# MDFahimAnjum/AliasFree-Diffusion-Models-PyTorch

Measured on AMD Instinct MI355X. Metric: train_step_images_per_sec, higher is better.
Workload: dtype f32; 1 GPU; CIFAR-10 32x32x3 synthetic, UNet variant=3 (Config D), batch 256/GPU, T=1000, AdamW lr 3e-4, random-init weights (seed 42); global_batch=256, parallelism=dp1, hip_graph=True, launch_mode=lanes

## Files before the change

aliasfree-diffusion-models-pytorch_amd/csrc/conv.hip:

```cpp
#include <cstdlib>
#include <algorithm>
#include "common.h"

namespace afd {

using f32x16 = __attribute__((ext_vector_type(16))) float;

static inline int gs_grid(long total, int block = 256) {
  long g = (total + block - 1) / block;
  return (int)(g < 1 ? 1 : (g > 65536 ? 65536 : g));
}

template <int KS>
__global__ void conv_direct_fwd(const float* __restrict__ x, const float* __restrict__ w, const float* __restrict__ bias,
                                const float* __restrict__ res, float* __restrict__ y,
                                int Cin, int Cout, int H, int W, int act, long total) {
  constexpr int T = KS * KS, R = KS / 2;
  for (long i = blockIdx.x * (long)blockDim.x + threadIdx.x; i < total; i += (long)gridDim.x * blockDim.x) {
    const int xx = i % W, yy = (i / W) % H;
    const long bc = i / ((long)W * H);
    const int co = bc % Cout; const long b = bc / Cout;
    float acc = bias ? bias[co] : 0.f;
    for (int ci = 0; ci < Cin; ++ci) {
      const float* xp = x + (b * Cin + ci) * (long)H * W;
// ... 564 lines not shown
    const int bn = threadIdx.x >> 2;
    if ((threadIdx.x & 3) == 0 && bn < BNo && n0 + bn < Cout) bias_part[(long)split * Cout + n0 + bn] = t;
  }
  float* out = part + (long)split * Cout * Cin * T;
  if (WK == 1) {
    if (!active) return;
    const int ci = c0 + cw + l31;
    if (ci < Cin) {
#pragma unroll
      for (int r = 0; r < 16; ++r) {
        const int n = n0 + nw + (r & 3) + 8 * (r >> 2) + 4 * half;
        if (n >= Cout) continue;
#pragma unroll
        for (int t = 0; t < T; ++t) out[((long)t * Cout + n) * Cin + ci] = acc[t][r];
      }
    }
  } else {
    float* red = smem;
    constexpr int NB = WNn * WCn;
#pragma unroll
    for (int t = 0; t < T; ++t) {
      __syncthreads();
#pragma unroll
      for (int r = 0; r < 16; ++r) red[(wv * 16 + r) * 64 + lane] = acc[t][r];
      __syncthreads();
      for (int idx = threadIdx.x; idx < NB * 1024; idx += NT_) {
        const int blk = idx / 1024, r = (idx / 64) % 16, ln = idx % 64;
        float v = 0.f;
#pragma unroll
        for (int k = 0; k < WK; ++k) v += red[((k * NB + blk) * 16 + r) * 64 + ln];
        const int bn = blk % WNn, bc = blk / WNn;
        const int n = n0 + bn * 32 + (r & 3) + 8 * (r >> 2) + 4 * (ln >> 5);
        const int ci = c0 + bc * 32 + (ln & 31);
        if (n < Cout && ci < Cin) out[((long)t * Cout + n) * Cin + ci] = v;
      }
    }
  }
}

__global__ __launch_bounds__(256) void wgrad_reduce(const float* __restrict__ part, float* __restrict__ dw, long n, int splits,
                                                    const float* __restrict__ bias_part, float* __restrict__ db, int nb,
                                                    int accumulate, int T) {
  __shared__ float red[8][33];
  const long i = (long)blockIdx.x * 32 + (threadIdx.x & 31);
  const int g = threadIdx.x >> 5;
  const bool isw = i < n;
  const long j = isw ? i : i - n;
  const long stride = isw ? n : nb;
  const float* __restrict__ src = isw ? part : bias_part;
  float s0 = 0.f, s1 = 0.f, s2 = 0.f, s3 = 0.f;
  if (i < n + nb) {
    int k = g;
    for (; k + 24 < splits; k += 32) {
      s0 += src[(long)k * stride + j]; s1 += src[(long)(k + 8) * stride + j];
      s2 += src[(long)(k + 16) * stride + j]; s3 += src[(long)(k + 24) * stride + j];
    }
    for (; k < splits; k += 8) s0 += src[(long)k * stride + j];
  }
  red[g][threadIdx.x & 31] = (s0 + s1) + (s2 + s3);
  __syncthreads();
  if (g == 0 && i < n + nb) {
    float t = 0.f;
#pragma unroll
    for (int k = 0; k < 8; ++k) t += red[k][threadIdx.x & 31];
    const long plane = n / T;
    float* o = isw ? dw + (j % plane) * T + j / plane : db + j;
    *o = accumulate ? *o + t : t;
  }
}

__global__ __launch_bounds__(256) void wgrad_reduce4(const float* __restrict__ part, float* __restrict__ dw, long n, int splits,
                                                     const float* __restrict__ bias_part, float* __restrict__ db, int nb,
                                                     int accumulate, int T) {
  __shared__ float4 red4[8][32];
  const int l = threadIdx.x & 31, g = threadIdx.x >> 5;
  const long wblocks = n >> 7;
  if (blockIdx.x < wblocks) {
    const long j = ((long)blockIdx.x << 7) + 4 * l;
    const float4* __restrict__ src = reinterpret_cast<const float4*>(part + j);
    const long stride = n >> 2;
    float4 s0 = {0.f, 0.f, 0.f, 0.f}, s1 = s0, s2 = s0, s3 = s0;
    int k = g;
    for (; k + 24 < splits; k += 32) {
      const float4 a = src[(long)k * stride], b = src[(long)(k + 8) * stride], c = src[(long)(k + 16) * stride],
                   d = src[(long)(k + 24) * stride];
      s0.x += a.x; s0.y += a.y; s0.z += a.z; s0.w += a.w;
      s1.x += b.x; s1.y += b.y; s1.z += b.z; s1.w += b.w;
      s2.x += c.x; s2.y += c.y; s2.z += c.z; s2.w += c.w;
      s3.x += d.x; s3.y += d.y; s3.z += d.z; s3.w += d.w;
    }
    for (; k < splits; k += 8) {
      const float4 a = src[(long)k * stride];
      s0.x += a.x; s0.y += a.y; s0.z += a.z; s0.w += a.w;
    }
    red4[g][l] = make_float4((s0.x + s1.x) + (s2.x + s3.x), (s0.y + s1.y) + (s2.y + s3.y), (s0.z + s1.z) + (s2.z + s3.z),
                             (s0.w + s1.w) + (s2.w + s3.w));
    __syncthreads();
    if (threadIdx.x < 128) {
      const int e = threadIdx.x;
      float t = 0.f;
#pragma unroll
      for (int q = 0; q < 8; ++q) t += reinterpret_cast<const float*>(&red4[q][e >> 2])[e & 3];
      const long je = ((long)blockIdx.x << 7) + e, plane = n / T;
      float* o = dw + (je % plane) * T + je / plane;
      *o = accumulate ? *o + t : t;
    }
  } else {
    __shared__ float red[8][33];
    const long j = (long)(blockIdx.x - wblocks) * 32 + l;
    float s0 = 0.f;
    if (j < nb)
      for (int k = g; k < splits; k += 8) s0 += bias_part[(long)k * nb + j];
    red[g][l] = s0;
    __syncthreads();
    if (g == 0 && j < nb) {
      float t = 0.f;
#pragma unroll
      for (int q = 0; q < 8; ++q) t += red[q][l];
      db[j] = accumulate ? db[j] + t : t;
    }
  }
}

int fold_launch(const afd_fold_desc* descs, int n, hipStream_t s);

struct FoldSink { afd_fold_desc* out; int n; };
static int launch_wgrad_reduce(const float* part, float* dw, long n, int slabs, const float* bp, float* db, int nb, int accumulate,
                               int T, hipStream_t s, FoldSink* sink) {
  afd_fold_desc d[2];
  int nd = 0;
  d[nd++] = afd_fold_desc{part, dw, n, n, n / T, (long)T, slabs, accumulate};
  if (nb > 0) d[nd++] = afd_fold_desc{bp, db, (long)nb, (long)nb, (long)nb, 1L, slabs, accumulate};
  if (sink) {
    for (int i = 0; i < nd; ++i) sink->out[sink->n++] = d[i];
    return AFD_OK;
  }
  return fold_launch(d, nd, s);
}

bool pw_launch(const float* in, const float* w, const float* bias, const float* res, float* out, int B, int K, int N, int P,
               int act, bool dgrad, hipStream_t s);
void pw_set_mode(int m);
int wino_plan(int B, int K, int N, int H, int W);
bool wino_conv(const float* x, const float* w, const float* bias, const float* res, float* y, float* U, int B, int K, int N, int H,
               int W, int act, bool dgrad, bool weights_ready, hipStream_t s);
void wino_set_mode(int m);
void wino_weights_launch(const float* w, float* Uf, float* Ud, int Cin, int Cout, int kinds, hipStream_t s);
bool bf3_ok(int B, int K, int N, int H, int W);
void bf3_set_mode(int m);
void direct_form_set(int m);
bool direct_form_is_bf3();
void h2_sk_set_mode(int m);
void h2_lds_set(int m);
void wino_weights_batched_launch(const afd_wino_desc* descs, const int* wg_desc, int n_wg, hipStream_t s);
void wino_set_grid(int g);
int wgrad_wino_plan(int B, int Cin, int Cout, int H, int W, int* bn, int* bk, int* cps, int* nchunks);
int wgrad_bf3_plan(int B, int Cin, int Cout, int H, int W, int* tps, int* ntiles);
int wgrad_bf3(const float* x, const float* dy, float* part, int B, int Cin, int Cout, int H, int W, hipStream_t s);
void wgrad_bf3_set_mode(int m);
void wgrad_arith_set(int m);
void wgrad_plan_target_set(long wgs);
bool wgrad_arith_is_bf3();
int wgrad_h2(const float* x, const float* dy, float* part, int B, int Cin, int Cout, int H, int W, hipStream_t s);
int pw_wgrad_h2(const float* x, const float* dy, float* part, float* bias_part, int B, int Cin, int Cout, int L, hipStream_t s);
bool ends_fwd(const float* x, const float* w, const float* bias, const float* res, float* y, int B, int Cin, int Cout, int H, int W,
              int ksize, int act, hipStream_t s);
bool ends_dgrad(const float* dy, const float* w, float* dx, int B, int Cin, int Cout, int H, int W, int ksize, hipStream_t s);
void ends_set_mode(int m);
int wgrad_cin3_plan(int B, int Cin, int Cout, int H, int W);
int wgrad_cin3(const float* x, const float* dy, float* part, int B, int Cin, int Cout, int H, int W, hipStream_t s);
void pw_wgrad_bf3_set_mode(int m);
int pw_wgrad_bf3_plan(int B, int Cin, int Cout, int L, int* sps, int* nsteps, int* nr, int* nt);
int pw_wgrad_bf3(const float* x, const float* dy, float* part, float* bias_part, int B, int Cin, int Cout, int L, hipStream_t s);
int wgrad_wino(const float* x, const float* dy, float* part, int B, int Cin, int Cout, int H, int W, hipStream_t s);
void wgrad_wino_set_mode(int m);

static inline bool use_mfma(int K, int N, int H, int W, int PT) { return N >= 8 && tile_ok(H, W, PT); }

static int g_conv_path = 0;

template <int T, bool DGRAD>
static int launch_mfma(const float* x, const float* w, const float* bias, const float* res, float* y,
                       int B, int K, int N, int H, int W, int act, hipStream_t s) {
  constexpr int KC = (T == 9) ? 8 : 32;
  const long P = (long)B * H * W;
  if (P * K >= (1L << 31) || (long)K * N * T >= (1L << 31)) return -1;
  const unsigned ptiles = (unsigned)((P + 127) / 128);
  const long wgs64 = (long)ptiles * ((N + 63) / 64), wgs32 = (long)ptiles * ((N + 31) / 32);
  bool use32 = N <= 32 || (wgs64 < 256 && wgs32 >= 256);
  const bool want_sk = g_conv_path == 2 || (g_conv_path == 0 && wgs64 < 256 && wgs32 < 256);
  if (g_conv_path == 1) use32 = N <= 32;
  if (want_sk && K >= 32 && tile_ok(H, W, 64)) {
    const TileGeom g = make_geom(H, W, 64, T == 9 ? 1 : 0);
    if (g.XS <= 256) {
      const size_t lds_main = sizeof(float) * (32 * (32 * T + 1) + (size_t)32 * g.XS);
      const size_t lds_red = sizeof(float) * 4 * 2 * 16 * 64;
      const size_t lds = lds_main > lds_red ? lds_main : lds_red;
      hipLaunchKernelGGL((conv_mfma_sk<T, DGRAD>), dim3((N + 31) / 32, (unsigned)((P + 63) / 64)), dim3(256), lds, s,
                         x, w, bias, res, y, B, K, N, H, W, act, g);
      return 0;
    }
  }
  const TileGeom g = make_geom(H, W, 128, T == 9 ? 1 : 0);
  if (g.XS > 512) return -1;
  int geo = 0;
  if (T == 1) geo = 5;
  else if (H == W && (W == 32 || W == 16 || W == 8 || W == 4)) geo = W == 32 ? 1 : (W == 16 ? 2 : (W == 8 ? 3 : 4));
  const size_t lds = 2 * sizeof(float) * ((use32 ? 32 : 64) * (KC * T + 1) + (size_t)KC * g.XS);
  const dim3 grid(use32 ? (N + 31) / 32 : (N + 63) / 64, ptiles);
#define AFD_CONV_LAUNCH(BN_, GEO_) hipLaunchKernelGGL((conv_mfma<T, DGRAD, BN_, KC, GEO_>), grid, dim3(256), lds, s, x, w, bias, res, y, B, K, N, H, W, act, g)
#define AFD_CONV_GEO(BN_)                                             \
  switch (geo) {                                                       \
    case 1: if constexpr (T == 9) { AFD_CONV_LAUNCH(BN_, 1); } break;  \
    case 2: if constexpr (T == 9) { AFD_CONV_LAUNCH(BN_, 2); } break;  \
    case 3: if constexpr (T == 9) { AFD_CONV_LAUNCH(BN_, 3); } break;  \
    case 4: if constexpr (T == 9) { AFD_CONV_LAUNCH(BN_, 4); } break;  \
    case 5: if constexpr (T == 1) { AFD_CONV_LAUNCH(BN_, 5); } break;  \
    default: AFD_CONV_LAUNCH(BN_, 0);                                  \
  }
  if (!use32) { AFD_CONV_GEO(64) } else { AFD_CONV_GEO(32) }
#undef AFD_CONV_GEO
#undef AFD_CONV_LAUNCH
  return 0;
}

static int g_wgrad_nw = 0;
struct WgradPlan { int wnn, wcn, wk, splits, slabs, nchunks, cps, npb; };
static inline WgradPlan wgrad_plan(int B, int Cin, int Cout, int H, int W, int ksize) {
  WgradPlan p;
  p.wnn = Cout > 32 ? 2 : 1;
  p.wcn = Cin > 32 ? 2 : 1;
  p.wk = 4 / (p.wnn * p.wcn);
  p.nchunks = (int)(((long)B * H * W + 63) / 64);
  const long tiles = (long)((Cout + 32 * p.wnn - 1) / (32 * p.wnn)) * ((Cin + 32 * p.wcn - 1) / (32 * p.wcn));
  static const long target = [] { const char* e = getenv("AFD_WG_TARGET"); return e ? atol(e) : 256L; }();
  long s = target / tiles;
  if (s < 1) s = 1;
  if (s > p.nchunks) s = p.nchunks;
  p.cps = (int)((p.nchunks + s - 1) / s);
  p.splits = (int)((p.nchunks + p.cps - 1) / p.cps);
  p.slabs = p.splits;
  const TileGeom g = make_geom(H, W, 64, ksize == 3 ? 1 : 0);
  const int need = (g.XS + 31) / 32;
  p.npb = ksize == 1 ? 2 : (need <= 4 ? 4 : (need <= 5 ? 5 : 8));
  return p;
}

template <int T, int WNn, int WCn, int NPB>
static void launch_wgrad(const float* x, const float* dy, float* part, float* bias_part, int B, int Cin, int Cout, int H, int W,
                         const WgradPlan& p, const TileGeom& g, hipStream_t s) {
  const int nw = g_wgrad_nw ? g_wgrad_nw : ((p.cps >= 8 || (p.cps >= 4 && H * W >= 256)) ? 8 : 4);
  size_t lds = sizeof(float) * ((size_t)32 * WNn * 65 + (size_t)32 * WCn * (g.XS | 1)) + sizeof(int) * 64;
  const size_t red = sizeof(float) * nw * 16 * 64;
  if (WNn * WCn < nw && lds < red) lds = red;
  const dim3 grid((Cout + 32 * WNn - 1) / (32 * WNn), (Cin + 32 * WCn - 1) / (32 * WCn), p.splits);
  if (nw == 8)
    hipLaunchKernelGGL((conv_wgrad_mfma<T, WNn, WCn, NPB, 8>), grid, dim3(512), lds, s, x, dy, part, bias_part, B, Cin, Cout, H, W, p.cps, p.nchunks, g);
  else
    hipLaunchKernelGGL((conv_wgrad_mfma<T, WNn, WCn, NPB, 4>), grid, dim3(256), lds, s, x, dy, part, bias_part, B, Cin, Cout, H, W, p.cps, p.nchunks, g);
}

template <int T, int NPB>
static void launch_wgrad_roles(const float* x, const float* dy, float* part, float* bp, int B, int Cin, int Cout, int H, int W,
                               const WgradPlan& p, const TileGeom& g, hipStream_t s) {
  if (p.wnn == 2 && p.wcn == 2) launch_wgrad<T, 2, 2, NPB>(x, dy, part, bp, B, Cin, Cout, H, W, p, g, s);
  else if (p.wnn == 2) launch_wgrad<T, 2, 1, NPB>(x, dy, part, bp, B, Cin, Cout, H, W, p, g, s);
  else if (p.wcn == 2) launch_wgrad<T, 1, 2, NPB>(x, dy, part, bp, B, Cin, Cout, H, W, p, g, s);
  else launch_wgrad<T, 1, 1, NPB>(x, dy, part, bp, B, Cin, Cout, H, W, p, g, s);
}

}
using namespace afd;

extern "C" {

int afd_debug_conv_path(int mode) {
  if (mode >= 92 && mode <= 93) { ends_set_mode(mode - 92); return AFD_OK; }
  if (mode >= 88 && mode <= 89) { pw_wgrad_bf3_set_mode(mode - 88); return AFD_OK; }
  if (mode >= 84 && mode <= 86) { wgrad_bf3_set_mode(mode - 84); return AFD_OK; }
  if (mode >= 48 && mode <= 49) { wgrad_plan_target_set(mode == 48 ? 256 : 160); return AFD_OK; }
  if (mode >= 59 && mode <= 63) { h2_lds_set(mode == 59 ? 4 : (mode == 60 ? 1 : (mode == 61 ? 0 : mode - 60))); return AFD_OK; }
  if (mode == 73) { h2_sk_set_mode(2); return AFD_OK; }
  if (mode >= 74 && mode <= 75) { h2_sk_set_mode(mode - 74); return AFD_OK; }
  if (mode >= 78 && mode <= 79) { wgrad_arith_set(mode - 78); return AFD_OK; }
  if (mode >= 76 && mode <= 77) { direct_form_set(mode - 76); return AFD_OK; }
  if (mode >= 80 && mode <= 82) { bf3_set_mode(mode - 80); return AFD_OK; }
  if (mode >= 8 && mode <= 10) { pw_set_mode(mode - 8); return AFD_OK; }
  if (mode >= 100000 && mode < 200000) { wino_set_grid(mode - 100000); return AFD_OK; }
  if (mode >= 96 && mode <= 98) { wgrad_wino_set_mode(mode - 96); return AFD_OK; }
  if (mode >= 64 && mode <= 70) { wino_set_mode(mode - 64); return AFD_OK; }
  if (mode >= 32 && mode <= 34) { g_wgrad_nw = mode == 32 ? 4 : (mode == 33 ? 8 : 0); return AFD_OK; }
  AFD_REQUIRE(mode >= 0 && mode <= 2, "afd_debug_conv_path: mode must be 0 (auto), 1 (big tile), 2 (split-K tile), 8..10 (1x1 streaming auto/off/forced), 32..34 (wgrad waves 4/8/auto), 64..69 (Winograd fwd/dgrad auto/off/forced shapes) or 96..98 (Winograd wgrad auto/off/forced)");
  g_conv_path = mode;
  return AFD_OK;
}

int afd_conv_fwd(const float* x, const float* w, const float* bias, const float* res, float* y,
                 int B, int Cin, int Cout, int H, int W, int ksize, int act, afd_stream_t st) {
  AFD_REQUIRE(x && w && y && B > 0 && Cin > 0 && Cout > 0 && H > 0 && W > 0, "afd_conv_fwd: bad argument");
  AFD_REQUIRE(ksize == 1 || ksize == 3, "afd_conv_fwd: ksize %d not in {1,3}", ksize);
  AFD_REQUIRE(act == 0 || act == 1, "afd_conv_fwd: act must be 0 or 1");
  hipStream_t s = as_stream(st);
  if (ends_fwd(x, w, bias, res, y, B, Cin, Cout, H, W, ksize, act, s)) return check_launch("afd_conv_fwd");
  if (ksize == 1 && pw_launch(x, w, bias, res, y, B, Cin, Cout, H * W, act, false, s)) return check_launch("afd_conv_fwd");
  int rc = -1;
  if (use_mfma(Cin, Cout, H, W, 128))
    rc = ksize == 3 ? launch_mfma<9, false>(x, w, bias, res, y, B, Cin, Cout, H, W, act, s)
                    : launch_mfma<1, false>(x, w, bias, res, y, B, Cin, Cout, H, W, act, s);
  if (rc != 0) {
    const long total = (long)B * Cout * H * W;
    if (ksize == 3) hipLaunchKernelGGL(conv_direct_fwd<3>, dim3(gs_grid(total)), dim3(256), 0, s, x, w, bias, res, y, Cin, Cout, H, W, act, total);
    else hipLaunchKernelGGL(conv_direct_fwd<1>, dim3(gs_grid(total)), dim3(256), 0, s, x, w, bias, res, y, Cin, Cout, H, W, act, total);
  }
  return check_launch("afd_conv_fwd");
}

int afd_conv_dgrad(const float* dy, const float* w, float* dx, int B, int Cin, int Cout, int H, int W, int ksize, afd_stream_t st) {
  AFD_REQUIRE(dy && w && dx && B > 0 && Cin > 0 && Cout > 0 && H > 0 && W > 0, "afd_conv_dgrad: bad argument");
  AFD_REQUIRE(ksize == 1 || ksize == 3, "afd_conv_dgrad: ksize %d not in {1,3}", ksize);
  hipStream_t s = as_stream(st);
  if (ends_dgrad(dy, w, dx, B, Cin, Cout, H, W, ksize, s)) return check_launch("afd_conv_dgrad");
  if (ksize == 1 && pw_launch(dy, w, nullptr, nullptr, dx, B, Cout, Cin, H * W, 0, true, s)) return check_launch("afd_conv_dgrad");
  int rc = -1;
  if (use_mfma(Cout, Cin, H, W, 128))
    rc = ksize == 3 ? launch_mfma<9, true>(dy, w, nullptr, nullptr, dx, B, Cout, Cin, H, W, 0, s)
                    : launch_mfma<1, true>(dy, w, nullptr, nullptr, dx, B, Cout, Cin, H, W, 0, s);
  if (rc != 0) {
    const long total = (long)B * Cin * H * W;
    if (ksize == 3) hipLaunchKernelGGL(conv_direct_dgrad<3>, dim3(gs_grid(total)), dim3(256), 0, s, dy, w, dx, Cin, Cout, H, W, total);
    else hipLaunchKernelGGL(conv_direct_dgrad<1>, dim3(gs_grid(total)), dim3(256), 0, s, dy, w, dx, Cin, Cout, H, W, total);
  }
  return check_launch("afd_conv_dgrad");
}

size_t afd_conv3x3_wino_workspace_bytes(int B, int Cin, int Cout, int H, int W, int dgrad) {
  if (B <= 0 || Cin <= 0 || Cout <= 0 || H <= 0 || W <= 0) return 0;
  const int K = dgrad ? Cout : Cin, N = dgrad ? Cin : Cout;
  return (bf3_ok(B, K, N, H, W) || wino_plan(B, K, N, H, W)) ? sizeof(float) * 16 * (size_t)Cin * Cout : 0;
}

int afd_conv3x3_weight_kinds(int B, int Cin, int Cout, int H, int W) {
  if (B <= 0 || Cin <= 0 || Cout <= 0 || H <= 0 || W <= 0) return 0;
  const int k = (bf3_ok(B, Cin, Cout, H, W) ? 1 : 0) | (bf3_ok(B, Cout, Cin, H, W) ? 2 : 0);
  return k && direct_form_is_bf3() ? k | 4 : k;
}

int afd_conv3x3_wino_weights(const float* w, float* u_fwd, float* u_dgrad, int Cin, int Cout, int kinds, afd_stream_t st) {
  AFD_REQUIRE(w && (u_fwd || u_dgrad) && Cin > 0 && Cout > 0 && Cin % 8 == 0 && Cout % 8 == 0, "afd_conv3x3_wino_weights: bad argument");
  AFD_REQUIRE(kinds >= 0 && kinds <= 7 && (!(kinds & 4) || (kinds & 3)) && (!(kinds & 3) || (Cin % 16 == 0 && Cout % 16 == 0)), "afd_conv3x3_wino_weights: bad kinds %d", kinds);
  wino_weights_launch(w, u_fwd, u_dgrad, Cin, Cout, kinds, as_stream(st));
  return check_launch("afd_conv3x3_wino_weights");
}

int afd_conv3x3_wino_weights_batched(const afd_wino_desc* descs, const int* wg_desc, int n_wg, afd_stream_t st) {
  AFD_REQUIRE(descs && wg_desc && n_wg > 0, "afd_conv3x3_wino_weights_batched: bad argument");
  wino_weights_batched_launch(descs, wg_desc, n_wg, as_stream(st));
  return check_launch("afd_conv3x3_wino_weights_batched");
}

static int check_kinds(const char* who, int kinds, int B, int Cin, int Cout, int H, int W, int dgrad) {
  const int now = afd_conv3x3_weight_kinds(B, Cin, Cout, H, W);
  const int bit = dgrad ? 2 : 1;
  AFD_REQUIRE(kinds >= 0 && (kinds & bit) == (now & bit) && (!(now & bit) || (kinds & 4) == (now & 4)),
              "%s: the weight image was built as kinds %d, but a call with (B %d, %d -> %d, %dx%d) under the current settings reads kinds %d "
              "(rebuild it: afd_conv3x3_weight_kinds depends on the batch size and on afd_debug_conv_path)", who, kinds, B, Cin, Cout, H, W, now);
  return AFD_OK;
}

int afd_conv3x3_wino_fwd(const float* x, const float* w, const float* bias, const float* res, float* y,
                         int B, int Cin, int Cout, int H, int W, int act, void* workspace, int weights_ready, int kinds, afd_stream_t st) {
  AFD_REQUIRE(x && w && y && workspace && B > 0 && Cin > 0 && Cout > 0 && H > 0 && W > 0, "afd_conv3x3_wino_fwd: bad argument");
  AFD_REQUIRE(act == 0 || act == 1, "afd_conv3x3_wino_fwd: act must be 0 or 1");
  if (weights_ready && check_kinds("afd_conv3x3_wino_fwd", kinds, B, Cin, Cout, H, W, 0) != AFD_OK) return AFD_EINVAL;
  AFD_REQUIRE(wino_conv(x, w, bias, res, y, static_cast<float*>(workspace), B, Cin, Cout, H, W, act, false, weights_ready != 0, as_stream(st)),
              "afd_conv3x3_wino_fwd: shape (%d,%d->%d,%dx%d) is not covered (afd_conv3x3_wino_workspace_bytes returns 0 for it)", B, Cin, Cout, H, W);
  return check_launch("afd_conv3x3_wino_fwd");
}

int afd_conv3x3_wino_dgrad(const float* dy, const float* w, float* dx, const float* add_to_dx, int B, int Cin, int Cout, int H, int W,
                           void* workspace, int weights_ready, int kinds, afd_stream_t st) {
  AFD_REQUIRE(dy && w && dx && workspace && B > 0 && Cin > 0 && Cout > 0 && H > 0 && W > 0, "afd_conv3x3_wino_dgrad: bad argument");
  if (weights_ready && check_kinds("afd_conv3x3_wino_dgrad", kinds, B, Cin, Cout, H, W, 1) != AFD_OK) return AFD_EINVAL;
  AFD_REQUIRE(wino_conv(dy, w, nullptr, add_to_dx, dx, static_cast<float*>(workspace), B, Cout, Cin, H, W, 0, true, weights_ready != 0, as_stream(st)),
              "afd_conv3x3_wino_dgrad: shape (%d,%d->%d,%dx%d) is not covered", B, Cin, Cout, H, W);
  return check_launch("afd_conv3x3_wino_dgrad");
}

size_t afd_conv_wgrad_workspace_bytes(int B, int Cin, int Cout, int H, int W, int ksize) {
  if (B <= 0 || Cin <= 0 || Cout <= 0 || H <= 0 || W <= 0) return 0;
  size_t pw = 0;
  if (ksize == 1) {
    int a, b, c, d;
    pw = sizeof(float) * (size_t)pw_wgrad_bf3_plan(B, Cin, Cout, H * W, &a, &b, &c, &d) * ((size_t)Cout * Cin + Cout);
  }
  if (!tile_ok(H, W, 64)) return std::max(pw, sizeof(float) * (size_t)B * Cout);
  size_t slabs = wgrad_plan(B, Cin, Cout, H, W, ksize).slabs;
  if (ksize == 3) {
    int bn, bk, cps, nch;
    const size_t ws = (size_t)wgrad_wino_plan(B, Cin, Cout, H, W, &bn, &bk, &cps, &nch);
    if (ws > slabs) slabs = ws;
    const size_t wb = (size_t)wgrad_bf3_plan(B, Cin, Cout, H, W, &cps, &nch);
    if (wb > slabs) slabs = wb;
    const size_t wc = (size_t)wgrad_cin3_plan(B, Cin, Cout, H, W);
    if (wc > slabs) slabs = wc;
  }
  const size_t need = slabs * ((size_t)Cout * Cin * ksize * ksize + Cout);
  const size_t direct = (size_t)B * Cout;
  return std::max(pw, sizeof(float) * (need > direct ? need : direct));
}

int afd_conv_wgrad_form(int B, int Cin, int Cout, int H, int W, int ksize) {
  if (B <= 0 || Cin <= 0 || Cout <= 0 || H <= 0 || W <= 0) return 0;
  int a, b, c, d;
  if (ksize == 1) return pw_wgrad_bf3_plan(B, Cin, Cout, H * W, &a, &b, &c, &d) ? (wgrad_arith_is_bf3() ? 2 : 4) : 0;
  if (ksize != 3) return 0;
  if (wgrad_bf3_plan(B, Cin, Cout, H, W, &a, &b)) return wgrad_arith_is_bf3() ? 2 : 4;
  if (wgrad_cin3_plan(B, Cin, Cout, H, W)) return 3;
  return wgrad_wino_plan(B, Cin, Cout, H, W, &a, &b, &c, &d) ? 1 : 0;
}

static int conv_wgrad_impl(const float* x, const float* dy, float* dw, float* dbias, int B, int Cin, int Cout, int H, int W,
                           int ksize, int accumulate, void* workspace, FoldSink* sink, hipStream_t s, const char* who) {
  AFD_REQUIRE(x && dy && dw && B > 0 && Cin > 0 && Cout > 0 && H > 0 && W > 0, "%s: bad argument", who);
  AFD_REQUIRE(ksize == 1 || ksize == 3, "%s: ksize %d not in {1,3}", who, ksize);
  const int T = ksize * ksize;
  const TileGeom g = make_geom(H, W, 64, ksize == 3 ? 1 : 0);
  int rc = AFD_OK;
  if (ksize == 3 && !dbias && workspace) {
    float* part = static_cast<float*>(workspace);
    int slabs = wgrad_arith_is_bf3() ? wgrad_bf3(x, dy, part, B, Cin, Cout, H, W, s) : wgrad_h2(x, dy, part, B, Cin, Cout, H, W, s);
    if (!slabs) slabs = wgrad_cin3(x, dy, part, B, Cin, Cout, H, W, s);
    if (!slabs) slabs = wgrad_wino(x, dy, part, B, Cin, Cout, H, W, s);
    if (slabs) {
      const long n = (long)Cout * Cin * 9;
      rc = launch_wgrad_reduce(part, dw, n, slabs, nullptr, nullptr, 0, accumulate, 9, s, sink);
      return rc != AFD_OK ? rc : check_launch(who);
    }
  }
  if (ksize == 1 && workspace) {
    int a, b, c, d;
    const int slabs = pw_wgrad_bf3_plan(B, Cin, Cout, H * W, &a, &b, &c, &d);
    if (slabs) {
      float* part = static_cast<float*>(workspace);
      const long n = (long)Cout * Cin;
      float* bp = dbias ? part + (size_t)slabs * n : nullptr;
// ... 49 lines not shown
```

aliasfree-diffusion-models-pytorch_amd/csrc/h2.hip:

```cpp
#include <algorithm>
#include <cstdint>
#include "common.h"
#include "h2_common.h"

namespace afd {

using f32x4 = __attribute__((ext_vector_type(4))) float;

#ifndef AFD_H2_ABL
#define AFD_H2_ABL 0
#endif
#ifndef AFD_H2_AQ
#define AFD_H2_AQ 2
#endif
#ifndef AFD_H2_PRIO
#define AFD_H2_PRIO 0
#endif
#ifndef AFD_H2_SLEEP
#define AFD_H2_SLEEP 0
#endif
#ifndef AFD_H2_LDSPAD
#define AFD_H2_LDSPAD 0
#endif
#ifndef AFD_H2_STAMP
// ... 302 lines not shown
      Xp[G::KG * NPP + s_dst[e]] = p1;
    }
  };

  const int K8 = K >> 3;
  int soff[CPW];
#pragma unroll
  for (int d = 0; d < CPW; ++d) {
    const int c = wv * CPW + d;
    const int pt = NT == 64 ? c >> 2 : c >> 1, kg = NT == 64 ? c & 3 : 2 * (c & 1) + lh, n = NT == 64 ? lane : l31;
    const int pc = pt / 3, tx = pt - 3 * pc;
    soff[d] = ((pc * 9 + tx) * K8 + kg) * N + n0w + n;
  }
  auto dma_row = [&](int q) {
    const int ks = q / 3, ty = q - 3 * ks;
    const h8* src = Wp + (long)(ty * 3 * K8 + 4 * ks) * N;
    h8* dst = Ab + (q & 1) * AROW + wv * CPW * 64;
#pragma unroll
    for (int d = 0; d < CPW; ++d)
      __builtin_amdgcn_global_load_lds((const __attribute__((address_space(1))) void*)(src + soff[d]),
                                       (__attribute__((address_space(3))) void*)(dst + d * 64), 16, 0, 0);
  };
#define AFD_ROW_END(younger)                                                                                              \
  do {                                                                                                                    \
    __builtin_amdgcn_sched_barrier(0);                                                                                    \
    __builtin_amdgcn_s_waitcnt(((younger) & 15) | 0x0F70 | (((younger) >> 4) << 14));                \
    asm volatile("" ::: "memory");                                                                                        \
    __builtin_amdgcn_s_barrier();                                                                                         \
    asm volatile("" ::: "memory");                                                                                        \
    __builtin_amdgcn_sched_barrier(0);                                                                                    \
  } while (0)

  dma_row(0);
  fetch(0);
  AFD_STAMP();

  int bbase[PB];
#pragma unroll
  for (int pb = 0; pb < PB; ++pb) {
    int i, r, c;
    G::pixel(pgrp * PB + pb, l31, i, r, c);
    bbase[pb] = lh * NPP + i * G::IMG + r * G::Wp + c;
  }
  const int abase = lh * NT + 32 * nb + l31;
  f32x16 acc[PB];
#pragma unroll
  for (int pb = 0; pb < PB; ++pb)
#pragma unroll
    for (int j = 0; j < 16; ++j) acc[pb][j] = 0.f;

  const int KS = K >> 5, nrows = 3 * KS;
  float sx = __uint_as_float(kH2ScaleCapBits);
  AFD_STAMP();
  int q = 0;
  for (int k0 = 0; k0 < K; k0 += 32) {
    chunk_amax();
    __builtin_amdgcn_sched_barrier(0);
    __builtin_amdgcn_s_waitcnt(0x0F70);
    __builtin_amdgcn_sched_barrier(0);
    if (k0 < 64) AFD_STAMP();
    __syncthreads();
    {
      const float m = fmaxf(fmaxf(wmax[0], wmax[1]), fmaxf(wmax[2], wmax[3]));
      const float sn = fminf(sx, h2_scale_for(m));
      if (sn != sx) {
        const float f = sn * h2_inv_pow2(sx);
#pragma unroll
        for (int pb = 0; pb < PB; ++pb) acc[pb] *= f;
        sx = sn;
      }
    }
    commit(sx);
    __syncthreads();
    if (k0 < 64) AFD_STAMP();
#pragma unroll
    for (int ty = 0; ty < 3; ++ty, ++q) {
      if (q + 1 < nrows) dma_row(q + 1);
      const bool prefetch = ty == 1 && k0 + 32 < K;
      if (prefetch) fetch(k0 + 32);
      const h8* Ar = Ab + (q & 1) * AROW + abase;
      constexpr int U = 3 * 2 * PB;
      h8 ac[2], an[2], bc[2], bn[2];
      ac[0] = Ar[0]; ac[1] = Ar[3 * 4 * NT];
      bc[0] = Xp[bbase[0] + ty * G::Wp]; bc[1] = Xp[G::KG * NPP + bbase[0] + ty * G::Wp];
#pragma unroll
      for (int u = 0; u < U; ++u) {
        const int pb = u % PB;
        if (u + 1 < U) {
          const int un = u + 1, txn = un / (2 * PB), khn = (un / PB) % 2, pbn = un % PB;
          if (pbn == 0) { an[0] = Ar[(txn * 4 + 2 * khn) * NT]; an[1] = Ar[((3 + txn) * 4 + 2 * khn) * NT]; }
          const int o = bbase[pbn] + ty * G::Wp + txn + 2 * khn * NPP;
          bn[0] = Xp[o]; bn[1] = Xp[G::KG * NPP + o];
        }
        __builtin_amdgcn_sched_barrier(0);
        acc[pb] = __builtin_amdgcn_mfma_f32_32x32x16_f16(ac[0], bc[0], acc[pb], 0, 0, 0);
        acc[pb] = __builtin_amdgcn_mfma_f32_32x32x16_f16(ac[1], bc[0], acc[pb], 0, 0, 0);
        acc[pb] = __builtin_amdgcn_mfma_f32_32x32x16_f16(ac[0], bc[1], acc[pb], 0, 0, 0);
        __builtin_amdgcn_sched_barrier(0);
        if (u + 1 < U) {
          if ((u + 1) % PB == 0) { ac[0] = an[0]; ac[1] = an[1]; }
          bc[0] = bn[0]; bc[1] = bn[1];
        }
      }
      if (ty == 0) AFD_ROW_END(0);
      if (ty == 1) { if (prefetch) AFD_ROW_END(NE * 8); else AFD_ROW_END(0); }
      if (k0 < 64) AFD_STAMP();
    }
  }

  const float* isw = reinterpret_cast<const float*>(reinterpret_cast<const uint8_t*>(Wp) + h2_scale_offset_bytes(K, N));
  const float isx = h2_inv_pow2(sx);
#if AFD_H2_STAMP
  si = 13;
#endif
  AFD_STAMP();
  __syncthreads();
  float* T = reinterpret_cast<float*>(smem_raw) + wv * (32 * 36);
  const int cn = lane >> 3, cm = lane & 7;
  float sw[4], bv[4];
#pragma unroll
  for (int it = 0; it < 4; ++it) { sw[it] = isw[n0 + 8 * it + cn]; bv[it] = bias ? bias[n0 + 8 * it + cn] : 0.f; }
#pragma unroll
  for (int pb = 0; pb < PB; ++pb) {
#pragma unroll
    for (int j = 0; j < 16; ++j) T[(8 * (j >> 2) + 4 * lh + (j & 3)) * 36 + l31] = acc[pb][j] * isx;
    int i, r, c;
    G::pixel(pgrp * PB + pb, 4 * cm, i, r, c);
    const int b = img0 + i;
#pragma unroll
    for (int it = 0; it < 4; ++it) {
      const int nn = n0 + 8 * it + cn;
      f32x4 v = *reinterpret_cast<const f32x4*>(T + (8 * it + cn) * 36 + 4 * cm);
      if (b >= B) continue;
      const long o = ((long)b * N + nn) * HW + (row0 + r) * S + c;
#pragma unroll
      for (int e = 0; e < 4; ++e) {
        float u = v[e] * sw[it] + bv[it];
        if (act == 1) u = gelu_erf(u);
        v[e] = u;
      }
      if (res) v += *reinterpret_cast<const f32x4*>(res + o);
      *reinterpret_cast<f32x4*>(y + o) = v;
    }
  }
  AFD_STAMP();
#undef AFD_STAMP
}

template <int S> struct SkGeo {
  static constexpr int IPS = S == 4 ? 2 : 1;
  static constexpr int R = 32 / (IPS * S);
  static constexpr int Wp = S + 2, IMG = (R + 2) * Wp, NPIX = IPS * IMG, NPP = (NPIX + 15) / 16 * 16;
  static constexpr int KG = 4, TASKS = KG * NPIX, NE = (TASKS + 63) / 64;
};

template <int S, int KSP>
__global__ __launch_bounds__(256, 2) void conv_h2_sk(const float* __restrict__ x, const h8* __restrict__ Wp,
                                                     const float* __restrict__ bias, const float* __restrict__ res,
                                                     float* __restrict__ y, int B, int K, int N, int act, int nslices) {
  using G = SkGeo<S>;
  constexpr int PSP = 4 / KSP, NPP = G::NPP, NE = G::NE, HW = S * S;
  extern __shared__ __attribute__((aligned(16))) uint8_t smem_raw[];
  const int tid = threadIdx.x, lane = tid & 63, wv = tid >> 6, kgl = lane >> 4, l15 = lane & 15;
  const int kw = wv % KSP, pw = wv / KSP;
  h8* Xw = reinterpret_cast<h8*>(smem_raw) + (size_t)wv * 2 * G::KG * NPP;
  float* red = reinterpret_cast<float*>(smem_raw + (size_t)4 * 2 * G::KG * NPP * 16);
  const int sl = blockIdx.x * PSP + pw, n0 = blockIdx.y * 32;
  const bool live = sl < nslices;
  const int img0 = S == 4 ? sl * 2 : sl / 2, row0 = S == 4 ? 0 : (sl & 1) * 4;

  int s_src[NE], s_dst[NE];
#pragma unroll
  for (int e = 0; e < NE; ++e) {
    const int t = lane + 64 * e;
    s_src[e] = -1; s_dst[e] = -1;
    if (t < G::TASKS) {
      const int kg = t / G::NPIX, ridx = t - kg * G::NPIX;
      const int i = ridx / G::IMG, rem = ridx - i * G::IMG, rr = rem / G::Wp, cc = rem - rr * G::Wp;
      const int yy = row0 + rr - 1, xx = cc - 1, b = img0 + i;
      s_dst[e] = kg * NPP + ridx;
      if (live && yy >= 0 && yy < S && xx >= 0 && xx < S && b < B) s_src[e] = ((i * K + 8 * kg) * S + yy) * S + xx;
    }
  }
  const float* xb = x + (long)(live ? img0 : 0) * K * HW;
  float xr[NE][8];
  auto fetch = [&](int k0) {
#pragma unroll
    for (int e = 0; e < NE; ++e) {
      const float* p = xb + (long)k0 * HW + (s_src[e] >= 0 ? s_src[e] : 0);
#pragma unroll
      for (int j = 0; j < 8; ++j) xr[e][j] = s_src[e] >= 0 ? p[(long)j * HW] : 0.f;
    }
  };
  int bbase[2];
#pragma unroll
  for (int ps = 0; ps < 2; ++ps) {
    const int q = ps * 16 + l15;
    const int i = q / (G::R * S), rem = q - i * (G::R * S), r = rem / S, c = rem - r * S;
    bbase[ps] = kgl * NPP + i * G::IMG + r * G::Wp + c;
  }
  f32x4 acc[2][2];
#pragma unroll
  for (int ns = 0; ns < 2; ++ns)
#pragma unroll
    for (int ps = 0; ps < 2; ++ps) acc[ns][ps] = f32x4{0.f, 0.f, 0.f, 0.f};

  const int KS = K >> 5;
  const long pstride = (long)9 * (K >> 3) * N;
  const h8* wl = Wp + (long)kgl * N + n0 + l15;
  float sx = __uint_as_float(kH2ScaleCapBits);
  if (kw < KS) fetch(32 * kw);
  for (int ks = kw; ks < KS; ks += KSP) {
    h8 ac[3][2][2], an[3][2][2];
    auto a_row = [&](h8 (&a)[3][2][2], int ty) {
#pragma unroll
      for (int tx = 0; tx < 3; ++tx) {
        const long r = ((long)(ty * 3 + tx) * (K >> 3) + 4 * ks) * N;
#pragma unroll
        for (int ns = 0; ns < 2; ++ns) { a[tx][ns][0] = wl[r + 16 * ns]; a[tx][ns][1] = wl[pstride + r + 16 * ns]; }
      }
    };
    a_row(ac, 0);
    {
      float m = 0.f;
#pragma unroll
      for (int e = 0; e < NE; ++e)
#pragma unroll
        for (int j = 0; j < 8; ++j) m = fmaxf(m, fabsf(xr[e][j]));
      const float sn = fminf(sx, h2_scale_for(wave_amax(m)));
      if (sn != sx) {
        const float f = sn * h2_inv_pow2(sx);
#pragma unroll
        for (int ns = 0; ns < 2; ++ns)
#pragma unroll
          for (int ps = 0; ps < 2; ++ps) acc[ns][ps] *= f;
        sx = sn;
      }
    }
#pragma unroll
    for (int e = 0; e < NE; ++e) {
      if (s_dst[e] < 0) continue;
      h8 p0, p1;
      h2_split8(xr[e], sx, p0, p1);
      Xw[s_dst[e]] = p0;
      Xw[G::KG * NPP + s_dst[e]] = p1;
    }
    if (ks + KSP < KS) fetch(32 * (ks + KSP));
#pragma unroll
    for (int ty = 0; ty < 3; ++ty) {
      if (ty < 2) a_row(an, ty + 1);
      __builtin_amdgcn_sched_barrier(0);
#pragma unroll
      for (int tx = 0; tx < 3; ++tx) {
#pragma unroll
        for (int ps = 0; ps < 2; ++ps) {
          const int o = bbase[ps] + ty * G::Wp + tx;
          const h8 b0 = Xw[o], b1 = Xw[G::KG * NPP + o];
#pragma unroll
          for (int ns = 0; ns < 2; ++ns) {
            acc[ns][ps] = __builtin_amdgcn_mfma_f32_16x16x32_f16(ac[tx][ns][0], b0, acc[ns][ps], 0, 0, 0);
            acc[ns][ps] = __builtin_amdgcn_mfma_f32_16x16x32_f16(ac[tx][ns][1], b0, acc[ns][ps], 0, 0, 0);
            acc[ns][ps] = __builtin_amdgcn_mfma_f32_16x16x32_f16(ac[tx][ns][0], b1, acc[ns][ps], 0, 0, 0);
          }
        }
      }
      __builtin_amdgcn_sched_barrier(0);
      if (ty < 2) {
#pragma unroll
        for (int tx = 0; tx < 3; ++tx)
#pragma unroll
          for (int ns = 0; ns < 2; ++ns) { ac[tx][ns][0] = an[tx][ns][0]; ac[tx][ns][1] = an[tx][ns][1]; }
      }
    }
  }
  {
    const float isx = h2_inv_pow2(sx);
#pragma unroll
    for (int ns = 0; ns < 2; ++ns)
#pragma unroll
      for (int ps = 0; ps < 2; ++ps)
#pragma unroll
        for (int rg = 0; rg < 4; ++rg) red[(wv * 16 + (ns * 2 + ps) * 4 + rg) * 64 + lane] = acc[ns][ps][rg] * isx;
  }
  __syncthreads();
  if (kw != 0 || !live) return;
  const float* isw = reinterpret_cast<const float*>(reinterpret_cast<const uint8_t*>(Wp) + h2_scale_offset_bytes(K, N));
#pragma unroll
  for (int ps = 0; ps < 2; ++ps) {
    const int q = ps * 16 + l15;
    const int i = q / (G::R * S), rem = q - i * (G::R * S), r = rem / S, c = rem - r * S;
    const int b = img0 + i;
    if (b >= B) continue;
#pragma unroll
    for (int ns = 0; ns < 2; ++ns) {
      const int nn = n0 + 16 * ns + 4 * kgl;
      const long o = ((long)b * N + nn) * HW + (row0 + r) * S + c;
#pragma unroll
      for (int rg = 0; rg < 4; ++rg) {
        float v = 0.f;
#pragma unroll
        for (int g = 0; g < KSP; ++g) v += red[((pw * KSP + g) * 16 + (ns * 2 + ps) * 4 + rg) * 64 + lane];
        v *= isw[nn + rg];
        if (bias) v += bias[nn + rg];
        if (act == 1) v = gelu_erf(v);
        if (res) v += res[o + (long)rg * HW];
        y[o + (long)rg * HW] = v;
      }
    }
  }
}

static int h2_nblk(long tiles, int N, int S) {
  static const long minwg = [] { const char* e = getenv("AFD_H2_MINWG"); return e ? atol(e) : 512L; }();
  for (int nb = S == 16 ? 4 : 2; nb > 1; nb >>= 1)
    if (N % (32 * nb) == 0 && tiles * (N / (32 * nb)) >= minwg) return nb;
  return 1;
}

void h2_weights_launch(const float* w, void* Wf, void* Wd, int Cin, int Cout, hipStream_t s) {
  const int rows = (Wf ? Cout : 0) + (Wd ? Cin : 0);
  hipLaunchKernelGGL(h2_wscale, dim3((unsigned)((rows + 3) / 4)), dim3(256), 0, s, w, Wf, Wd, Cin, Cout);
  hipLaunchKernelGGL(h2_weights, dim3((unsigned)((Cin * Cout / 64 + 3) / 4)), dim3(256), 0, s, w, Wf, Wd, Cin, Cout);
}

template <int S, int NBLK>
static void h2_launch_t(const float* x, const void* Wp, const float* bias, const float* res, float* y, int B, int K, int N, int act,
                        hipStream_t s) {
  using G = H2Geo<S>;
  const size_t lds = (size_t)2 * G::KG * G::NPP * 16 + 16;
  const long tiles = G::IPT > 1 ? ((long)B + G::IPT - 1) / G::IPT : (long)B * G::TPI;
  hipLaunchKernelGGL((conv_h2<S, NBLK>), dim3((unsigned)tiles, (unsigned)(N / (32 * NBLK))), dim3(256), lds, s, x,
                     static_cast<const h8*>(Wp), bias, res, y, B, K, N, act);
}
template <int S, int KSP>
static void h2_sk_launch_t(const float* x, const void* Wp, const float* bias, const float* res, float* y, int B, int K, int N, int act,
                           hipStream_t s) {
  using G = SkGeo<S>;
  const size_t lds = (size_t)4 * 2 * G::KG * G::NPP * 16 + sizeof(float) * 4 * 16 * 64;
  const int nslices = (int)(((long)B * S * S + 31) / 32), psp = 4 / KSP;
  hipLaunchKernelGGL((conv_h2_sk<S, KSP>), dim3((unsigned)((nslices + psp - 1) / psp), (unsigned)(N / 32)), dim3(256), lds, s, x,
                     static_cast<const h8*>(Wp), bias, res, y, B, K, N, act, nslices);
}
bool h2_sk_ok(int B, int K, int N, int H, int W, bool force) {
  if (H != W || (W != 4 && W != 8) || K % 32 || N % 32 || K < 64) return false;
  if ((long)B * K * H * W >= (1L << 31) || (long)B * N * H * W >= (1L << 31)) return false;
  if (force) return true;
  const long slices = ((long)B * H * W + 31) / 32;
  const int ksp = K >= 128 ? 4 : 2;
  return ((slices + 4 / ksp - 1) / (4 / ksp)) * (N / 32) >= 128;
}
static int g_h2_lds = 1;
void h2_lds_set(int m) { g_h2_lds = m; }
template <int S, int TP, int NB>
static int h2l_launch_t(const float* x, const void* Wp, const float* bias, const float* res, float* y, int B, int K, int N, int act,
                        hipStream_t s) {
  using G = H2LGeo<S, TP>;
  const size_t lds = (size_t)(2 * G::KG * G::NPP + 2 * 2 * 3 * 4 * 32 * NB) * 16 + 16 + AFD_H2_LDSPAD;
  if (int rc = lds_opt_in(conv_h2l<S, TP, NB>, lds)) return rc;
  const long tiles = G::IPT > 1 ? ((long)B + G::IPT - 1) / G::IPT : (long)B * G::TPI;
  hipLaunchKernelGGL((conv_h2l<S, TP, NB>), dim3((unsigned)tiles, (unsigned)(N / (32 * NB))), dim3(256), lds, s, x,
                     static_cast<const h8*>(Wp), bias, res, y, B, K, N, act);
  return AFD_OK;
}
template <int S>
static int h2l_launch(const float* x, const void* Wp, const float* bias, const float* res, float* y, int B, int K, int N, int act,
                      hipStream_t s) {
  const long px = (long)B * S * S;
  if (g_h2_lds != 4 && N % 64 == 0 && (g_h2_lds == 2 || (g_h2_lds == 1 && ((px + 127) / 128) * (N / 64) >= 512)))
    return h2l_launch_t<S, 128, 2>(x, Wp, bias, res, y, B, K, N, act, s);
  if constexpr (S >= 16) {
    if (g_h2_lds == 3 || (g_h2_lds == 1 && ((px + 255) / 256) * (N / 32) >= 512)) return h2l_launch_t<S, 256, 1>(x, Wp, bias, res, y, B, K, N, act, s);
  }
  return h2l_launch_t<S, 128, 1>(x, Wp, bias, res, y, B, K, N, act, s);
}

void h2_conv(const float* x, const void* Wp, const float* bias, const float* res, float* y, int B, int K, int N, int S, int act,
             hipStream_t s, bool small) {
  if (small) {
    if (S == 4) { if (K >= 128) h2_sk_launch_t<4, 4>(x, Wp, bias, res, y, B, K, N, act, s); else h2_sk_launch_t<4, 2>(x, Wp, bias, res, y, B, K, N, act, s); }
    else { if (K >= 128) h2_sk_launch_t<8, 4>(x, Wp, bias, res, y, B, K, N, act, s); else h2_sk_launch_t<8, 2>(x, Wp, bias, res, y, B, K, N, act, s); }
    return;
  }
  if (g_h2_lds > 1 || (g_h2_lds == 1 && S == 32 && N % 64 != 0)) {
    if (S == 32) h2l_launch<32>(x, Wp, bias, res, y, B, K, N, act, s);
    else if (S == 16) h2l_launch<16>(x, Wp, bias, res, y, B, K, N, act, s);
    else h2l_launch<8>(x, Wp, bias, res, y, B, K, N, act, s);
    return;
  }
  const int nblk = h2_nblk(((long)B * S * S + 127) / 128, N, S);
#define AFD_H2(S_)                                                                      \
  if (nblk == 4 && S_ == 16) h2_launch_t<16, 4>(x, Wp, bias, res, y, B, K, N, act, s);  \
  else if (nblk == 2) h2_launch_t<S_, 2>(x, Wp, bias, res, y, B, K, N, act, s);         \
  else h2_launch_t<S_, 1>(x, Wp, bias, res, y, B, K, N, act, s)
  if (S == 32) { AFD_H2(32); } else if (S == 16) { AFD_H2(16); } else { AFD_H2(8); }
#undef AFD_H2
}

}
```

Baseline: 38150 images/s.

## Process multiple pixel slices per wave in split-K small-image h2 conv

```diff
diff --git a/aliasfree-diffusion-models-pytorch_amd/csrc/conv.hip b/aliasfree-diffusion-models-pytorch_amd/csrc/conv.hip
--- a/aliasfree-diffusion-models-pytorch_amd/csrc/conv.hip
+++ b/aliasfree-diffusion-models-pytorch_amd/csrc/conv.hip
@@ -740,6 +740,7 @@
 bool direct_form_is_bf3();
 void h2_sk_set_mode(int m);
 void h2_lds_set(int m);
+void h2_sk_set_ppw(int m);
 void wino_weights_batched_launch(const afd_wino_desc* descs, const int* wg_desc, int n_wg, hipStream_t s);
 void wino_set_grid(int g);
 int wgrad_wino_plan(int B, int Cin, int Cout, int H, int W, int* bn, int* bk, int* cps, int* nchunks);
@@ -868,6 +869,7 @@
   if (mode >= 84 && mode <= 86) { wgrad_bf3_set_mode(mode - 84); return AFD_OK; }
   if (mode >= 48 && mode <= 49) { wgrad_plan_target_set(mode == 48 ? 256 : 160); return AFD_OK; }
   if (mode >= 59 && mode <= 63) { h2_lds_set(mode == 59 ? 4 : (mode == 60 ? 1 : (mode == 61 ? 0 : mode - 60))); return AFD_OK; }
+  if (mode >= 50 && mode <= 54 && mode != 53) { h2_sk_set_ppw(mode - 50); return AFD_OK; }
   if (mode == 73) { h2_sk_set_mode(2); return AFD_OK; }
   if (mode >= 74 && mode <= 75) { h2_sk_set_mode(mode - 74); return AFD_OK; }
   if (mode >= 78 && mode <= 79) { wgrad_arith_set(mode - 78); return AFD_OK; }
@@ -878,7 +880,7 @@
   if (mode >= 96 && mode <= 98) { wgrad_wino_set_mode(mode - 96); return AFD_OK; }
   if (mode >= 64 && mode <= 70) { wino_set_mode(mode - 64); return AFD_OK; }
   if (mode >= 32 && mode <= 34) { g_wgrad_nw = mode == 32 ? 4 : (mode == 33 ? 8 : 0); return AFD_OK; }
-  AFD_REQUIRE(mode >= 0 && mode <= 2, "afd_debug_conv_path: mode must be 0 (auto), 1 (big tile), 2 (split-K tile), 8..10 (1x1 streaming auto/off/forced), 32..34 (wgrad waves 4/8/auto), 64..69 (Winograd fwd/dgrad auto/off/forced shapes) or 96..98 (Winograd wgrad auto/off/forced)");
+  AFD_REQUIRE(mode >= 0 && mode <= 2, "afd_debug_conv_path: mode must be 0 (auto), 1 (big tile), 2 (split-K tile), 8..10 (1x1 streaming auto/off/forced), 32..34 (wgrad waves 4/8/auto), 50..52 / 54 (split-K 3x3 slices per wave auto/1/2/4), 64..69 (Winograd fwd/dgrad auto/off/forced shapes) or 96..98 (Winograd wgrad auto/off/forced)");
   g_conv_path = mode;
   return AFD_OK;
 }
diff --git a/aliasfree-diffusion-models-pytorch_amd/csrc/h2.hip b/aliasfree-diffusion-models-pytorch_amd/csrc/h2.hip
--- a/aliasfree-diffusion-models-pytorch_amd/csrc/h2.hip
+++ b/aliasfree-diffusion-models-pytorch_amd/csrc/h2.hip
@@ -478,15 +478,15 @@
   static constexpr int R = 32 / (IPS * S);
   static constexpr int Wp = S + 2, IMG = (R + 2) * Wp, NPIX = IPS * IMG, NPP = (NPIX + 15) / 16 * 16;
   static constexpr int KG = 4, TASKS = KG * NPIX, NE = (TASKS + 63) / 64;
+  static constexpr int IMGR = 2 * KG * NPP - (NPP - NPIX);
 };
 
 template <int S, int KSP>
-__global__ __launch_bounds__(256, 2) void conv_h2_sk(const float* __restrict__ x, const h8* __restrict__ Wp,
-                                                     const float* __restrict__ bias, const float* __restrict__ res,
-                                                     float* __restrict__ y, int B, int K, int N, int act, int nslices) {
+__device__ __forceinline__ void sk_one(uint8_t* smem_raw, const float* __restrict__ x, const h8* __restrict__ Wp,
+                                       const float* __restrict__ bias, const float* __restrict__ res,
+                                       float* __restrict__ y, int B, int K, int N, int act, int nslices) {
   using G = SkGeo<S>;
   constexpr int PSP = 4 / KSP, NPP = G::NPP, NE = G::NE, HW = S * S;
-  extern __shared__ __attribute__((aligned(16))) uint8_t smem_raw[];
   const int tid = threadIdx.x, lane = tid & 63, wv = tid >> 6, kgl = lane >> 4, l15 = lane & 15;
   const int kw = wv % KSP, pw = wv / KSP;
   h8* Xw = reinterpret_cast<h8*>(smem_raw) + (size_t)wv * 2 * G::KG * NPP;
@@ -636,6 +636,196 @@
   }
 }
 
+#ifndef AFD_SK_NA
+#define AFD_SK_NA 3
+#endif
+#ifndef AFD_SK_XB
+#define AFD_SK_XB 2
+#endif
+template <int S, int KSP, int PPW>
+__device__ __forceinline__ void sk_wide(uint8_t* smem_raw, const float* __restrict__ x, const h8* __restrict__ Wp,
+                                        const float* __restrict__ bias, const float* __restrict__ res,
+                                        float* __restrict__ y, int B, int K, int N, int act) {
+  using G = SkGeo<S>;
+  constexpr int PSP = 4 / KSP, NPP = G::NPP, NE = G::NE, HW = S * S;
+  constexpr int IMGR = G::IMGR;
+  constexpr int NA = AFD_SK_NA, XB = AFD_SK_XB < PPW ? AFD_SK_XB : PPW, NV = S == 8 ? 2 : 1;
+  static_assert(PPW % XB == 0 && NA >= 2 && NA <= 9 && IMGR * 16 >= 16 * 64 * 4, "conv_h2_sk: ring sizes");
+  const int tid = threadIdx.x, lane = tid & 63, wv = tid >> 6, kgl = lane >> 4, l15 = lane & 15;
+  const int kw = wv % KSP, pw = wv / KSP;
+  h8* Xw = reinterpret_cast<h8*>(smem_raw) + (size_t)wv * PPW * IMGR;
+  const int sl0 = (blockIdx.x * PSP + pw) * PPW, n0 = blockIdx.y * 32;
+  auto img_of = [&](int p) { return S == 4 ? (sl0 + p) * 2 : (sl0 + p) / 2; };
+
+  int s_src[NV][NE], s_dst[NE];
+#pragma unroll
+  for (int e = 0; e < NE; ++e) {
+    const int t = lane + 64 * e;
+    s_dst[e] = -1;
+#pragma unroll
+    for (int v = 0; v < NV; ++v) s_src[v][e] = -1;
+    if (t < G::TASKS) {
+      const int kg = t / G::NPIX, ridx = t - kg * G::NPIX;
+      const int i = ridx / G::IMG, rem = ridx - i * G::IMG, rr = rem / G::Wp, cc = rem - rr * G::Wp;
+      const int xx = cc - 1;
+      s_dst[e] = (kg * NPP + ridx) | (i << 16);
+#pragma unroll
+      for (int v = 0; v < NV; ++v) {
+        const int yy = 4 * v + rr - 1;
+        if (yy >= 0 && yy < S && xx >= 0 && xx < S) s_src[v][e] = ((i * K + 8 * kg) * S + yy) * S + xx;
+      }
+    }
+  }
+  float xr[XB][NE][8];
+  auto fetch = [&](float (&r)[NE][8], int k0, int p) {
+    const int b0 = img_of(p);
+    const float* xb = x + ((long)b0 * K + k0) * HW;
+#pragma unroll
+    for (int e = 0; e < NE; ++e) {
+      const int so = s_src[S == 8 ? (p & 1) : 0][e];
+      const bool ok = so >= 0 && b0 + (s_dst[e] >> 16) < B;
+      const float* q = xb + (ok ? so : 0);
+#pragma unroll
+      for (int j = 0; j < 8; ++j) r[e][j] = ok ? q[(long)j * HW] : 0.f;
+    }
+  };
+  int bbase[2];
+#pragma unroll
+  for (int ps = 0; ps < 2; ++ps) {
+    const int q = ps * 16 + l15;
+    const int i = q / (G::R * S), rem = q - i * (G::R * S), r = rem / S, c = rem - r * S;
+    bbase[ps] = kgl * NPP + i * G::IMG + r * G::Wp + c;
+  }
+  f32x4 acc[PPW][2][2];
+  float sx[PPW];
+#pragma unroll
+  for (int p = 0; p < PPW; ++p) {
+    sx[p] = __uint_as_float(kH2ScaleCapBits);
+#pragma unroll
+    for (int ns = 0; ns < 2; ++ns)
+#pragma unroll
+      for (int ps = 0; ps < 2; ++ps) acc[p][ns][ps] = f32x4{0.f, 0.f, 0.f, 0.f};
+  }
+
+  const int KS = K >> 5;
+  const long pstride = (long)9 * (K >> 3) * N;
+  const h8* wl = Wp + (long)kgl * N + n0 + l15;
+  if (kw < KS) {
+#pragma unroll
+    for (int p = 0; p < XB; ++p) fetch(xr[p], 32 * kw, p);
+  }
+  for (int ks = kw; ks < KS; ks += KSP) {
+    h8 a[NA][2][2];
+    auto a_tap = [&](int t) {
+      const long r = ((long)t * (K >> 3) + 4 * ks) * N;
+#pragma unroll
+      for (int ns = 0; ns < 2; ++ns) { a[t % NA][ns][0] = wl[r + 16 * ns]; a[t % NA][ns][1] = wl[pstride + r + 16 * ns]; }
+    };
+#pragma unroll
+    for (int t = 0; t < NA - 1; ++t) a_tap(t);
+#pragma unroll
+    for (int p = 0; p < PPW; ++p) {
+      float (&xp)[NE][8] = xr[p % XB];
+      float m = 0.f;
+#pragma unroll
+      for (int e = 0; e < NE; ++e)
+#pragma unroll
+        for (int j = 0; j < 8; ++j) m = fmaxf(m, fabsf(xp[e][j]));
+      const float sn = fminf(sx[p], h2_scale_for(wave_amax(m)));
+      if (sn != sx[p]) {
+        const float f = sn * h2_inv_pow2(sx[p]);
+#pragma unroll
+        for (int ns = 0; ns < 2; ++ns)
+#pragma unroll
+          for (int ps = 0; ps < 2; ++ps) acc[p][ns][ps] *= f;
+        sx[p] = sn;
+      }
+#pragma unroll
+      for (int e = 0; e < NE; ++e) {
+        if (s_dst[e] < 0) continue;
+        h8 p0, p1;
+        h2_split8(xp[e], sx[p], p0, p1);
+        Xw[p * IMGR + (s_dst[e] & 0xffff)] = p0;
+        Xw[p * IMGR + G::KG * NPP + (s_dst[e] & 0xffff)] = p1;
+      }
+      if (p + XB < PPW) fetch(xp, 32 * ks, p + XB);
+      else if (ks + KSP < KS) fetch(xp, 32 * (ks + KSP), p + XB - PPW);
+    }
+#pragma unroll
+    for (int t = 0; t < 9; ++t) {
+      const int ty = t / 3, tx = t - 3 * ty;
+      if (t + NA - 1 < 9) a_tap(t + NA - 1);
+      __builtin_amdgcn_sched_barrier(0);
+#pragma unroll
+      for (int p = 0; p < PPW; ++p) {
+#pragma unroll
+        for (int ps = 0; ps < 2; ++ps) {
+          const int o = p * IMGR + bbase[ps] + ty * G::Wp + tx;
+          const h8 b0 = Xw[o], b1 = Xw[G::KG * NPP + o];
+#pragma unroll
+          for (int ns = 0; ns < 2; ++ns) {
+            acc[p][ns][ps] = __builtin_amdgcn_mfma_f32_16x16x32_f16(a[t % NA][ns][0], b0, acc[p][ns][ps], 0, 0, 0);
+            acc[p][ns][ps] = __builtin_amdgcn_mfma_f32_16x16x32_f16(a[t % NA][ns][1], b0, acc[p][ns][ps], 0, 0, 0);
+            acc[p][ns][ps] = __builtin_amdgcn_mfma_f32_16x16x32_f16(a[t % NA][ns][0], b1, acc[p][ns][ps], 0, 0, 0);
+          }
+        }
+      }
+      __builtin_amdgcn_sched_barrier(0);
+    }
+  }
+#pragma unroll
+  for (int p = 0; p < PPW; ++p) {
+    const float isx = h2_inv_pow2(sx[p]);
+    float* red = reinterpret_cast<float*>(Xw + p * IMGR);
+#pragma unroll
+    for (int ns = 0; ns < 2; ++ns)
+#pragma unroll
+      for (int ps = 0; ps < 2; ++ps)
+#pragma unroll
+        for (int rg = 0; rg < 4; ++rg) red[((ns * 2 + ps) * 4 + rg) * 64 + lane] = acc[p][ns][ps][rg] * isx;
+  }
+  __syncthreads();
+  if (kw != 0) return;
+  const float* isw = reinterpret_cast<const float*>(reinterpret_cast<const uint8_t*>(Wp) + h2_scale_offset_bytes(K, N));
+#pragma unroll
+  for (int p = 0; p < PPW; ++p) {
+    const int b0 = img_of(p), row0 = S == 4 ? 0 : (p & 1) * 4;
+    const float* redp = reinterpret_cast<const float*>(reinterpret_cast<const h8*>(smem_raw) + ((size_t)pw * KSP * PPW + p) * IMGR);
+#pragma unroll
+    for (int ps = 0; ps < 2; ++ps) {
+      const int q = ps * 16 + l15;
+      const int i = q / (G::R * S), rem = q - i * (G::R * S), r = rem / S, c = rem - r * S;
+      const int b = b0 + i;
+      if (b >= B) continue;
+#pragma unroll
+      for (int ns = 0; ns < 2; ++ns) {
+        const int nn = n0 + 16 * ns + 4 * kgl;
+        const long o = ((long)b * N + nn) * HW + (row0 + r) * S + c;
+#pragma unroll
+        for (int rg = 0; rg < 4; ++rg) {
+          float v = 0.f;
+#pragma unroll
+          for (int g = 0; g < KSP; ++g) v += redp[(size_t)g * PPW * IMGR * 4 + ((ns * 2 + ps) * 4 + rg) * 64 + lane];
+          v *= isw[nn + rg];
+          if (bias) v += bias[nn + rg];
+          if (act == 1) v = gelu_erf(v);
+          if (res) v += res[o + (long)rg * HW];
+          y[o + (long)rg * HW] = v;
+        }
+      }
+    }
+  }
+}
+
+template <int S, int KSP, int PPW>
+__global__ __launch_bounds__(256, PPW == 4 ? 1 : 2) void conv_h2_sk(const float* __restrict__ x, const h8* __restrict__ Wp,
+                                                                    const float* __restrict__ bias, const float* __restrict__ res,
+                                                                    float* __restrict__ y, int B, int K, int N, int act, int nslices) {
+  extern __shared__ __attribute__((aligned(16))) uint8_t smem_raw[];
+  if constexpr (PPW == 1) sk_one<S, KSP>(smem_raw, x, Wp, bias, res, y, B, K, N, act, nslices);
+  else sk_wide<S, KSP, PPW>(smem_raw, x, Wp, bias, res, y, B, K, N, act);
+}
+
 static int h2_nblk(long tiles, int N, int S) {
   static const long minwg = [] { const char* e = getenv("AFD_H2_MINWG"); return e ? atol(e) : 512L; }();
   for (int nb = S == 16 ? 4 : 2; nb > 1; nb >>= 1)
@@ -658,13 +848,15 @@
   hipLaunchKernelGGL((conv_h2<S, NBLK>), dim3((unsigned)tiles, (unsigned)(N / (32 * NBLK))), dim3(256), lds, s, x,
                      static_cast<const h8*>(Wp), bias, res, y, B, K, N, act);
 }
-template <int S, int KSP>
+template <int S, int KSP, int PPW>
 static void h2_sk_launch_t(const float* x, const void* Wp, const float* bias, const float* res, float* y, int B, int K, int N, int act,
                            hipStream_t s) {
   using G = SkGeo<S>;
-  const size_t lds = (size_t)4 * 2 * G::KG * G::NPP * 16 + sizeof(float) * 4 * 16 * 64;
-  const int nslices = (int)(((long)B * S * S + 31) / 32), psp = 4 / KSP;
-  hipLaunchKernelGGL((conv_h2_sk<S, KSP>), dim3((unsigned)((nslices + psp - 1) / psp), (unsigned)(N / 32)), dim3(256), lds, s, x,
+  const size_t lds = PPW == 1 ? (size_t)4 * 2 * G::KG * G::NPP * 16 + sizeof(float) * 4 * 16 * 64
+                              : (size_t)4 * PPW * G::IMGR * 16;
+  (void)lds_opt_in(&conv_h2_sk<S, KSP, PPW>, lds);
+  const int nslices = (int)(((long)B * S * S + 31) / 32), per = 4 / KSP * PPW;
+  hipLaunchKernelGGL((conv_h2_sk<S, KSP, PPW>), dim3((unsigned)((nslices + per - 1) / per), (unsigned)(N / 32)), dim3(256), lds, s, x,
                      static_cast<const h8*>(Wp), bias, res, y, B, K, N, act, nslices);
 }
 bool h2_sk_ok(int B, int K, int N, int H, int W, bool force) {
@@ -674,6 +866,14 @@
   const long slices = ((long)B * H * W + 31) / 32;
   const int ksp = K >= 128 ? 4 : 2;
   return ((slices + 4 / ksp - 1) / (4 / ksp)) * (N / 32) >= 128;
+}
+static int g_sk_ppw = 0;
+void h2_sk_set_ppw(int m) { g_sk_ppw = m; }
+static int h2_sk_ppw(int B, int K, int N, int S) {
+  if (g_sk_ppw) return g_sk_ppw;
+  const long slices = ((long)B * S * S + 31) / 32;
+  const int psp = K >= 128 ? 1 : 2;
+  return ((slices + psp - 1) / psp) * (N / 32) >= 1024 ? 2 : 1;
 }
 static int g_h2_lds = 1;
 void h2_lds_set(int m) { g_h2_lds = m; }
@@ -703,8 +903,14 @@
 void h2_conv(const float* x, const void* Wp, const float* bias, const float* res, float* y, int B, int K, int N, int S, int act,
              hipStream_t s, bool small) {
   if (small) {
-    if (S == 4) { if (K >= 128) h2_sk_launch_t<4, 4>(x, Wp, bias, res, y, B, K, N, act, s); else h2_sk_launch_t<4, 2>(x, Wp, bias, res, y, B, K, N, act, s); }
-    else { if (K >= 128) h2_sk_launch_t<8, 4>(x, Wp, bias, res, y, B, K, N, act, s); else h2_sk_launch_t<8, 2>(x, Wp, bias, res, y, B, K, N, act, s); }
+    const int ppw = h2_sk_ppw(B, K, N, S);
+#define AFD_SK(S_, KSP_)                                                                   \
+  if (ppw == 4) h2_sk_launch_t<S_, KSP_, 4>(x, Wp, bias, res, y, B, K, N, act, s);         \
+  else if (ppw == 2) h2_sk_launch_t<S_, KSP_, 2>(x, Wp, bias, res, y, B, K, N, act, s);    \
+  else h2_sk_launch_t<S_, KSP_, 1>(x, Wp, bias, res, y, B, K, N, act, s)
+    if (S == 4) { if (K >= 128) { AFD_SK(4, 4); } else { AFD_SK(4, 2); } }
+    else { if (K >= 128) { AFD_SK(8, 4); } else { AFD_SK(8, 2); } }
+#undef AFD_SK
     return;
   }
   if (g_h2_lds > 1 || (g_h2_lds == 1 && S == 32 && N % 64 != 0)) {
```

Result: no change. 38210 images/s, median of 3 (+0.2%).
